# SixLabors/ZlibStream

Measured on AMD Instinct MI355X. Metric: deflate MB/s (input) at level 6, 64 MiB buffers, higher is better.
Workload: dtype u8; 1 GPU; english64: 1 x 67108864-byte pseudo-random-English (Zipf words of alice29.txt) buffer per GPU, level 6, zlib framing, inputs resident in HBM; level=6, buffer_bytes=67108864, buffers_per_gpu=1, compressed_bytes=27425826, parallelism=independent buffers, 1 GPU(s), no collective in the data path

## Files before the change

### zlibstream_amd/csrc/zs_core.h

```cpp
#pragma once
#include <stdint.h>
#include <vector>

#if defined(__HIPCC__)
#include <hip/hip_runtime.h>
#define ZS_HD __host__ __device__ __forceinline__
#define ZS_HD_NOINLINE __host__ __device__
#else
#define ZS_HD inline
#define ZS_HD_NOINLINE
#endif

namespace zs {

constexpr int kMinMatch = 3;
constexpr int kMaxMatch = 258;
constexpr int kMinLookahead = kMaxMatch + kMinMatch + 1;
constexpr int kWSize = 32768;
constexpr int kWMask = kWSize - 1;
constexpr int kWindowSize = 2 * kWSize;
constexpr int kMaxDist = kWSize - kMinLookahead;
constexpr int kSlideAt = kWindowSize - kMinLookahead;
constexpr int kHashBits = 15;
constexpr int kHashSize = 1 << kHashBits;
// ... 836 lines not shown
        if (nextlen == 0) max_count = 138, min_count = 3;
        else if (curlen == nextlen) max_count = 6, min_count = 3;
        else max_count = 7, min_count = 4;
    }
}

template <class Put>
ZS_HD_NOINLINE inline void emit_dyn_header(const TreeWork &w, Put &put) {
    int lcodes = w.l_max_code + 1, dcodes = w.d_max_code + 1, blcodes = w.max_blindex + 1;
    put((unsigned)(lcodes - 257), 5);
    put((unsigned)(dcodes - 1), 5);
    put((unsigned)(blcodes - 4), 4);
    for (int rank = 0; rank < blcodes; rank++) put(w.bltree[bl_order(rank)].dl, 3);
    emit_tree_rle(w.ltree, lcodes - 1, w.bltree, put);
    emit_tree_rle(w.dtree, dcodes - 1, w.bltree, put);
}

ZS_HD unsigned zlib_header(int level) {
    unsigned header = (8u + (7u << 4)) << 8;
    unsigned lf = (((unsigned)(level - 1)) & 0xFF) >> 1;
    if (lf > 3) lf = 3;
    header |= lf << 6;
    header += 31 - (header % 31);
    return header;
}

constexpr uint32_t kAdlerBase = 65521;
ZS_HD uint32_t adler_combine(uint32_t a1, uint32_t a2, uint64_t len2) {
    uint32_t rem = (uint32_t)(len2 % kAdlerBase);
    uint32_t s1a = a1 & 0xFFFF, s2a = a1 >> 16, s1b = a2 & 0xFFFF, s2b = a2 >> 16;
// ... 173 lines not shown
```

### zlibstream_amd/csrc/zs_device.h

```cpp
#pragma once
#include <cstddef>
#include "zs_core.h"
#include "zs_lit_engine.h"
#include "zs_fast_sweep.h"
#include "zs_rle.h"

namespace zs {

constexpr int kMatchTile = 16384;
constexpr int kMatchBack = 32512;
constexpr int kMatchFwd = 272;
constexpr int kMatchLdsBytes = kMatchBack + kMatchTile + kMatchFwd;
constexpr int kMatchLdsLinks = kMatchBack + kMatchTile;
constexpr int kMatchLds = kMatchLdsBytes + 2 * kMatchLdsLinks;
constexpr int kAdlerPiece = 65536;

constexpr int64_t kScratchWindow = 0;
constexpr int64_t kScratchHead = 66560;
constexpr int64_t kScratchPrev = kScratchHead + 2 * kHashSize;
constexpr int64_t kScratchHead32 = kScratchPrev + 2 * kWSize;
constexpr int64_t kScratchBytes = kScratchHead32 + 4 * kHashSize;

struct StreamDesc {
    const uint8_t *in;
// ... 81 lines not shown
    uint32_t adler;
    int32_t status;
    int64_t end_bits;
    int32_t r_seg, r_slot, r_kfired, r_kslot;
    uint32_t r_total;
    int32_t r_ncut;
    int32_t r_cut_e[8], r_cut_done[8];
    int32_t deferred, r_scan;
    int32_t r_cutidx;
    int32_t nc[2], cuts_same, cut_diff_idx, cut_diff_pos;
    int32_t poison;
    int32_t spec_run_tiles, spec_ok, spec_wrong;
    int32_t body_bad;
    int64_t body_bits;
};
constexpr uint32_t kSpecBail = 1u << 30;
ZS_HD uint32_t spec_pack(int guess, int exit_slot, int count, bool bail) {
    return (uint32_t)guess | ((uint32_t)exit_slot << 9) | ((uint32_t)count << 18) | (bail ? kSpecBail : 0u);
}
ZS_HD int spec_guess(uint32_t r) { return (int)(r & 0x1FF); }
ZS_HD int spec_exit(uint32_t r) { return (int)((r >> 9) & 0x1FF); }
ZS_HD int spec_count(uint32_t r) { return (int)((r >> 18) & 0xFFF); }
constexpr int kSpecMinInput = 1 << 20;
constexpr int kSpecLenBits = 10;
constexpr int kSpecWarm = 128;
constexpr int kSpecRunsDen = 8;
struct K5Spec {
    uint32_t *rec;
    uint32_t *base;
    int len_bits, warm, corrupt;
// ... 32 lines not shown
```

### zlibstream_amd/csrc/zs_engine.hip

```cpp
#include <hip/hip_runtime.h>

#include <algorithm>
#include <cstdio>
#include <cstdlib>
#include <cstring>
#include <functional>
#include <string>
#include <thread>
#include <vector>

#define ZS_BUILDING_LIBRARY
#include "../../include/zsgpu.h"
#include "zs_kernels.hip"
#include "zs_inflate_par.hip"
#include "zs_inflate_tok.hip"
#include "zs_png.hip"
#include "zs_crc32.hip"
#include "zs_gzip.hip"
#include "zs_zip.hip"
#include "zs_tiff.hip"
#include "zs_exr.hip"
#include "zs_chunk.hip"
#include "zs_plan.h"

// ... 39 lines not shown
    int fast_fallbacks = 0;
    int round_runs = 0;
    int cut_rounds = 0;
    int lit_fallbacks = 0;
    int spec_streams = 0, spec_fallbacks = 0, spec_wrong_chunks = 0;
    int spec_periodic = 0;
    int64_t dbg_blk_off = 0, dbg_chunk_off = 0, dbg_nchunks = 0, dbg_spec_n = 0, dbg_n_spec = 0;
    int64_t lit_engine_bytes = 0;
    std::vector<int64_t> inf_used;
    int64_t *inf_probe = nullptr;
    int inf_lane_streams = 0;
    int inf_wave_streams = 0;
    int64_t png_segments = 0;
    int fast_rounds = 0;
    bool no_rounds_once = false;
    int last_op = 0;
    hipEvent_t ev[kStCount + 1] = {};
    double stage_ms[kStCount] = {};
    uint32_t *crc_tab = nullptr;
    DevBuf sd, st, work, link, mm, maps, chunk_far, segmap, supmap, seg_entry, seg_symbase, seg_stale, entry, symbase, stale, syms, blk_end, blk_top, blocks, trees, info, tile_bits, pieces, scratch,
        stage_in, stage_out, wr, inf_desc, inf_state, par_ps, par_st, par_work, par_cbits, par_ccnt, par_surv, par_scnt, par_cands, par_tabs, par_toktabs, par_toks, par_ctoks, par_tokstat, par_tails, par_retry, par_fxtab, par_blocks, par_cells,
        par_windows, par_fail, run_syms, run_bits, run_scratch, run_outs, run_fail, adl_tr, adl_res, plan_blk, ins_bits, mm_bak, cut_pos, cut_bkt, win_groups, win_sg, win_maps, win_entries, persist_bak, resume_flag, rle_tiles, own_in, fr_chunks, fr_meta, fr_planes, fr_prov, fr_base, fr_counters, spec_rec, spec_flags, spec_syms;
    uint32_t *crc32_tab = nullptr;
    DevBuf png[kBufPngCount];
    hipEvent_t ev_png[2] = {};
    bool resume_poisoned = false;
    void *pinned = nullptr;
    size_t pinned_cap = 0;
    void *pin_io = nullptr;
    size_t pin_io_cap = 0;
// ... 81 lines not shown
T *dev(DevBuf &b) {
    return (T *)b.p;
}


struct RunOpts : PlanRun {
    int64_t end_bits = 0;
};

struct LaunchEnv {
    bool no_plan_reuse = getenv("ZS_NO_PLAN_REUSE") != nullptr, no_supmap = getenv("ZS_NO_SUPMAP") != nullptr;
    bool no_defer = getenv("ZS_NO_DEFER") != nullptr, force_rounds = getenv("ZS_FORCE_ROUNDS") != nullptr;
    bool tail_serial = getenv("ZS_TAIL_SERIAL") != nullptr, tail_fork = getenv("ZS_TAIL_FORK") != nullptr, fast_no_probe = getenv("ZS_FAST_NO_PROBE") != nullptr;
    bool no_whole_runs = getenv("ZS_NO_WHOLE_RUNS") != nullptr, whole_runs = getenv("ZS_WHOLE_RUNS") != nullptr;
    bool no_split_backend = getenv("ZS_NO_SPLIT_BACKEND") != nullptr;
    bool debug = getenv("ZS_DEBUG") != nullptr, debug_cuts = getenv("ZS_DEBUG_CUTS") != nullptr, debug_fa = getenv("ZS_DEBUG_FA") != nullptr;
    const char *debug_chain = getenv("ZS_DEBUG_CHAIN"), *debug_chain_want = getenv("ZS_DEBUG_CHAIN_WANT");
    int k5_ahead = getenv("ZS_K5_AHEAD") ? atoi(getenv("ZS_K5_AHEAD")) : 1;
    int spec_corrupt = getenv("ZS_SPEC_CORRUPT") ? atoi(getenv("ZS_SPEC_CORRUPT")) : -1;
    static bool host_times() {
        static const bool v = getenv("ZS_HOST_TIMES") != nullptr;
        return v;
    }
    static const char *eb_tiles() {
        static const char *const v = getenv("ZS_EB_TILES");
        return v;
    }
};
struct RoundsEnv {
    int max_rounds = getenv("ZS_FR_MAX_ROUNDS") ? atoi(getenv("ZS_FR_MAX_ROUNDS")) : 0;
// ... 35 lines not shown
    LaunchEnv env;
    FoldedWrites folded;
    PlanArgs pa;
    bool any_writes = false, no_rounds_this_call = false, plan_hit = false, plan_keep = false;
    double ht_plan = 0, ht_launched = 0;
    const StreamDesc *d_sd = nullptr;
    StreamState *d_st = nullptr, *hst = nullptr;
    const uint2 *d_work = nullptr;
    bool prof = false;
    K5Spec k5s{};
    int spec_ok_streams = 0;
    bool need_maps = true, spec_ran = false;
    bool fork_recorded = false;
    bool tail_late = false, tail_serial = false, use_sup = false;
    bool split = false;
    int defer_mode = 0, cut_stride = 0;
    bool done = false, answer = false;

    double ht_us() const { return std::chrono::duration<double, std::micro>(std::chrono::steady_clock::now() - ht0).count(); }
    const uint2 *work(int list) const { return d_work + lay.work[list]; }
    void mark(int i) {
        if (prof) (void)hipEventRecord(c->ev[i], stream);
    }
    bool rerun(int force_seq_, bool rounds_, const std::vector<uint8_t> *force_lit_) {
        c->lit_engine_bytes -= pl.lit_bytes;
        done = true;
        return answer = run_pipeline(c, n, in, in_len, out, out_cap, out_len, status, level, strategy, hash_variant, stream, writes, force_seq_, ro, rounds_, force_lit_);
    }
    void launch_tail(hipStream_t on) {
        hipLaunchKernelGGL(zs_tail_kernel, dim3((unsigned)n), dim3(1024), kTailLds, on, d_sd, d_st, dev<uint16_t>(c->link),
// ... 37 lines not shown

bool DeflateCall::begin() {
    for (int i = 0; i < n; i++) {
        out_len[i] = 0;
        if (status) status[i] = ZS_STREAM_ERROR;
    }
    for (int i = 0; i < n && writes; i++) any_writes = any_writes || writes[i] != nullptr;
    if (any_writes && n > 1)
        for (int i = 0; i < n; i++)
            if (ro || (writes[i] && writes[i]->flushing())) {
                c->err = "flush modes and incremental runs take one stream a call";
                return false;
            }
    no_rounds_this_call = c->no_rounds_once;
    c->no_rounds_once = false;
    c->fast_rounds = 0;
    c->plan_reused = 0;
    bool flush_any = false;
    for (int i = 0; i < n && any_writes; i++)
        if (const WriteSpec *wr = writes[i]) flush_any = flush_any || wr->flushing() || wr->flush.size() != wr->ends.size();
    plan_keep = !ro && !rounds && !force_lit && !no_rounds_this_call && force_seq == 0 && level != 0 && !flush_any && !env.no_plan_reuse;
    if (plan_keep) {
        plan_key_fill(pc.probe, n, in_len, out_cap, level, strategy, hash_variant, force_seq, ro != nullptr, rounds, force_lit != nullptr, no_rounds_this_call,
                      any_writes ? writes : nullptr, penv);
        plan_hit = pc.valid && pc.gen == c->plan_gen && !pc.in_flight && plan_key_equal(pc.key, pc.probe);
    }
    if (!plan_hit) pc.valid = false, pc.dual_saved = false, c->plan_gen++;
    writes = fold_rle_writes(folded, n, in_len, writes, any_writes, level, strategy, ro != nullptr, penv);
    pa.n = n, pa.in = in, pa.in_len = in_len, pa.out = out, pa.out_cap = out_cap, pa.level = level, pa.strategy = strategy;
    pa.writes = writes, pa.force_seq = force_seq, pa.ro = ro, pa.rounds = rounds, pa.force_lit = force_lit, pa.no_rounds = no_rounds_this_call;
// ... 365 lines not shown
    };
    tiles([&](dim3 tg, int s0) { hipLaunchKernelGGL(zs_rle_starts_kernel, tg, dim3(256), 0, stream, d_sd, rt, s0); });
    hipLaunchKernelGGL(zs_rle_scan_kernel, dim3((unsigned)n), dim3(1024), 0, stream, d_sd, rt);
    tiles([&](dim3 tg, int s0) {
        hipLaunchKernelGGL(zs_rle_pass_kernel<0>, tg, dim3(256), 0, stream, d_sd, rt, dev<uint32_t>(c->syms), dev<int32_t>(c->blk_end), dev<int32_t>(c->blk_top), s0);
    });
    hipLaunchKernelGGL(zs_rle_sums_kernel, dim3((unsigned)n), dim3(1024), 0, stream, d_sd, d_st, rt);
    tiles([&](dim3 tg, int s0) {
        hipLaunchKernelGGL(zs_rle_pass_kernel<1>, tg, dim3(256), 0, stream, d_sd, rt, dev<uint32_t>(c->syms), dev<int32_t>(c->blk_end), dev<int32_t>(c->blk_top), s0);
    });
    return true;
}

bool DeflateCall::tails_and_symbols() {
    const bool beside_k5 = need_maps && (!pl.w_segs.empty() || !pl.w_chunks.empty());
    if (!tail_late && !tail_serial && (n < 64 || penv.no_live_list) && !env.no_split_backend && pl.n_runs == 0 && !beside_k5) {
        int64_t longest = 0;
        for (int i = 0; i < n; i++) longest = std::max(longest, in_len[i]);
        split = longest >= kBlockSyms;
    }
    if (!tail_late && !tail_serial) {
        if (!fork_recorded || need_maps) ZS_HIP(c, hipEventRecord(c->ev_fork, stream));
        ZS_HIP(c, hipStreamWaitEvent(c->aux, c->ev_fork, 0));
        launch_tail(c->aux);
        if (split && prof) (void)hipEventRecord(c->ev_part1[0], c->aux);
        if (!split) ZS_HIP(c, hipEventRecord(c->ev_join, c->aux));
    }
    if (!pl.w_segs.empty() && need_maps)
        hipLaunchKernelGGL(zs_expand_kernel, dim3((unsigned)((pl.w_segs.size() + 63) / 64)), dim3(64), 0, stream, d_sd, d_st,
                           work(kWSegs), (int)pl.w_segs.size(), dev<uint2>(c->mm), dev<uint16_t>(c->link),
                           dev<uint32_t>(c->maps), dev<uint16_t>(c->seg_entry), dev<uint32_t>(c->seg_symbase),
// ... 78 lines not shown
                       dev<uint32_t>(c->run_syms), dev<FastRunOut>(c->run_outs), dev<uint32_t>(c->syms), dev<int32_t>(c->blk_end),
                       dev<int32_t>(c->blk_top));
    hipLaunchKernelGGL(zs_fast_blocks_kernel, dim3((unsigned)n), dim3(64), 0, stream, d_sd, d_st, dev<FastRunOut>(c->run_outs),
                       dev<int32_t>(c->blk_end), dev<int32_t>(c->blk_top), dev<BlockRec>(c->blocks), n);
    return true;
}

bool DeflateCall::blocks_and_bits() {
    const int trees_threads = pl.w_blocks.size() > 8192 ? 128 : 256;
    if (n >= 64 && !penv.no_live_list) {
        int32_t *const d_live = (int32_t *)((uint8_t *)c->sd.p + lay.sd_bytes);
        hipLaunchKernelGGL(zs_live_scan_kernel, dim3(1), dim3(1024), 0, stream, d_st, n, d_live);
        hipLaunchKernelGGL(zs_live_fill_kernel, dim3((unsigned)((pl.w_blocks.size() + 255) / 256)), dim3(256), 0, stream, d_live, n,
                           (uint32_t)pl.w_blocks.size(), dev<uint2>(c->work) + lay.work[kWBlocks]);
    }
    auto trees = [&](hipStream_t on, int part) {
        hipLaunchKernelGGL(zs_trees_kernel, dim3((unsigned)pl.w_blocks.size()), dim3(trees_threads), 0, on, d_sd, d_st, work(kWBlocks), dev<uint32_t>(c->syms),
                           dev<BlockRec>(c->blocks), dev<TreeWork>(c->trees), dev<BlockInfo>(c->info), dev<int32_t>(c->tile_bits), strategy, level, part);
    };
    auto offsets = [&](hipStream_t on, int part) {
        hipLaunchKernelGGL(zs_offsets_kernel, dim3((unsigned)n), dim3(256), 0, on, d_sd, d_st, dev<BlockRec>(c->blocks), dev<BlockInfo>(c->info),
                           dev<TreeWork>(c->trees), dev<uint32_t>(c->pieces), level, n, part);
    };
    trees(stream, split ? kPartBody : kPartAll);
    mark(11);
    ZS_HIP(c, hipStreamWaitEvent(stream, c->ev_pre, 0));
    offsets(stream, split ? kPartBody : kPartAll);
    mark(12);
    if (split) ZS_HIP(c, hipEventRecord(c->ev_part0, stream));
    int eb_tiles = kEbTiles;
    if (level != 0) {
        int64_t longest = 0;
        for (int i = 0; i < n; i++) longest = std::max(longest, in_len[i]);
        eb_tiles = (int)std::min<int64_t>(kEbTiles, (longest + 1) / kEbTile + 1);
    }
    if (env.eb_tiles()) eb_tiles = std::max(1, std::min(kEbTiles, atoi(env.eb_tiles())));
    auto emit_bits = [&](hipStream_t on, int part) {
        hipLaunchKernelGGL(zs_emit_bits_kernel, dim3((unsigned)pl.w_blocks.size(), (unsigned)(1 + eb_tiles)), dim3(256), 0, on, d_sd, d_st, work(kWBlocks),
                           dev<uint32_t>(c->syms), dev<BlockRec>(c->blocks), dev<TreeWork>(c->trees), dev<BlockInfo>(c->info), dev<int32_t>(c->tile_bits), part);
    };
    emit_bits(stream, split ? kPartBody : kPartAll);
    mark(13);
    if (split) {
        trees(c->aux, kPartRest);
        ZS_HIP(c, hipStreamWaitEvent(c->aux, c->ev_part0, 0));
        offsets(c->aux, kPartRest);
        emit_bits(c->aux, kPartRest);
        if (prof) (void)hipEventRecord(c->ev_part1[1], c->aux);
        ZS_HIP(c, hipEventRecord(c->ev_join, c->aux));
        ZS_HIP(c, hipStreamWaitEvent(stream, c->ev_join, 0));
    }
    ZS_HIP(c, hipGetLastError());
    hst = (StreamState *)c->pinned;
    ZS_HIP(c, hipMemcpyAsync(hst, d_st, sizeof(StreamState) * (size_t)n, hipMemcpyDeviceToHost, stream));
// ... 77 lines not shown
                c->resume_poisoned = true;
                return false;
            }
            c->lit_fallbacks++;
            return rerun(force_seq, false, &fl);
        }
    }
    if (!ro && !rounds) {
        bool gave_up = false;
        for (int i = 0; i < n; i++) gave_up = gave_up || hst[i].deferred == 1;
        if (gave_up) {
            ZS_HIP(c, hipStreamSynchronize(c->aux));
            c->round_runs++;
            if (!run_cut_rounds()) return false;
            return rerun(force_seq, true, force_lit);
        }
    }
    if (ro) ro->end_bits = hst[0].end_bits;
    bool all_ok = true;
    for (int i = 0; i < n; i++) {
        out_len[i] = hst[i].out_len;
        if (status) status[i] = hst[i].status;
        if (hst[i].status != 0 && all_ok) {
            c->err = hst[i].status == ZS_BUF_ERROR ? "buffer error"
                                                   : "stored block larger than the reference's pending buffer (the managed engine throws here)";
            all_ok = false;
        }
    }
    return all_ok;
}
// ... 221 lines not shown
const char *zs_ctx_last_error(const zs_ctx *c) { return c ? c->err.c_str() : "no context"; }

int64_t zs_deflate_bound(int64_t n) { return n + (n >> 3) + 1024; }

void zs_ctx_set_profiling(zs_ctx *c, int enable) {
    if (c) c->profiling = enable != 0;
}
int zs_ctx_stage_count(const zs_ctx *) { return kStCount; }
int64_t zs_ctx_counter(const zs_ctx *c, const char *name) {
    if (!c || !name) return -1;
    const std::string k(name);
    if (k == "fast_rounds") return c->fast_rounds;
    if (k == "fast_fallbacks") return c->fast_fallbacks;
    if (k == "round_runs") return c->round_runs;
    if (k == "cut_rounds") return c->cut_rounds;
    if (k == "lit_fallbacks") return c->lit_fallbacks;
    if (k == "lit_engine_bytes") return c->lit_engine_bytes;
    if (k == "spec_streams") return c->spec_streams;
    if (k == "spec_fallbacks") return c->spec_fallbacks;
    if (k == "spec_periodic") return c->spec_periodic;
    if (k == "spec_wrong_chunks") return c->spec_wrong_chunks;
    if (k == "plan_reused") return c->plan_reused;
    if (k == "inf_lane_streams") return c->inf_lane_streams;
    if (k == "inf_wave_streams") return c->inf_wave_streams;
    if (k == "png_segments") return c->png_segments;
    return -1;
}

int64_t zs_ctx_debug_read(zs_ctx *c, const char *name, void *out, int64_t cap) {
    if (!c || !name || !out || !c->st.p) return -1;
// ... 787 lines not shown
```

### zlibstream_amd/csrc/zs_kernels.hip

```cpp
#include <hip/hip_runtime.h>

#include <type_traits>

#include "zs_device.h"
#include "zs_png.h"

namespace zs {

typedef uint32_t __attribute__((aligned(1))) u32u;
typedef uint64_t __attribute__((aligned(1))) u64u;
typedef const __attribute__((address_space(1))) uint8_t *gcbytes;
typedef __attribute__((address_space(1))) uint8_t *gbytes_w;
__device__ __forceinline__ gcbytes as_global(const uint8_t *p) { return (gcbytes)(uintptr_t)p; }
__device__ __forceinline__ gbytes_w as_global(uint8_t *p) { return (gbytes_w)(uintptr_t)p; }
typedef const __attribute__((address_space(1))) uint32_t __attribute__((aligned(1))) *gcu32u;
typedef const __attribute__((address_space(1))) uint64_t __attribute__((aligned(1))) *gcu64u;
__device__ __forceinline__ uint32_t g_u32_bytes(gcbytes p) {
    return (uint32_t)p[0] | ((uint32_t)p[1] << 8) | ((uint32_t)p[2] << 16) | ((uint32_t)p[3] << 24);
}
typedef uint32_t u32x4 __attribute__((ext_vector_type(4)));
typedef const __attribute__((address_space(1))) u32x4 *gcu32x4;
__device__ __forceinline__ uint32_t lds_u32(const uint8_t *base, int idx) {
    const uint32_t *q = (const uint32_t *)(base + (idx & ~3));
    return __builtin_amdgcn_alignbyte(q[1], q[0], (uint32_t)idx & 3u);
// ... 1979 lines not shown
    }
    if (cut < 0) return;
#pragma unroll
    for (int d = 32; d >= 1; d >>= 1) before += __shfl_xor(before, d, 64);
    if (lane != 0) return;
    const ChunkCtx cx = spec_chunk_ctx(s, c, sp.len_bits);
    const int64_t start = spec_first_start(cx.cs, spec_guess(r)) + before;
    const bool odd = cx.m != 0 && slab[sp.stride - 1] == (uint32_t)cut;
    const uint32_t bi = (base + (uint32_t)cut) / kBlockSyms;
    blk_end[s.blk_off + bi] = (int32_t)spec_sym_end(start, slab[cut]);
    blk_top[s.blk_off + bi] = (int32_t)spec_sym_top(start, odd);
}

enum { kPartAll = -1, kPartBody = 0, kPartRest = 1 };
__device__ __forceinline__ int stream_body_blocks(int part, const StreamDesc &s, const StreamState &ss) {
    if (part == kPartAll) return 0;
    const bool splits = s.wr_flush == nullptr && s.n_wr <= 1 && s.final_run && !s.resume && !s.cont && !s.cont_bits && s.fast_runs == 0 &&
                        s.plan_nblk == 0 && !ss.deferred;
    return splits ? (int)(ss.body_syms / kBlockSyms) : 0;
}

__global__ __launch_bounds__(256) void zs_body_blocks_kernel(const StreamDesc *sd, const StreamState *st, const int32_t *blk_end,
                                                             const int32_t *blk_top, BlockRec *blocks, uint32_t *syms, int part) {
    const StreamDesc s = sd[blockIdx.x];
    if (s.fast_runs > 0 || st[blockIdx.x].deferred) return;
    const int nb0 = stream_body_blocks(part, s, st[blockIdx.x]);
    if (part == kPartBody && nb0 == 0) return;
    if (s.resume)
        for (uint32_t i = threadIdx.x; i < s.start_syms; i += blockDim.x) syms[s.sym_off + i] = s.persist->syms[i];
    const int nb_body = (int)(st[blockIdx.x].body_syms / kBlockSyms);
    BlockRec *blk = blocks + s.blk_off;
    for (int i = threadIdx.x; i < (part == kPartRest && nb0 > 0 ? 0 : nb_body); i += blockDim.x) {
        int64_t start = i ? blk_end[s.blk_off + i - 1] : (s.resume ? s.start_block : 0);
        int64_t end = blk_end[s.blk_off + i];
// ... 735 lines not shown
    while (lo < hi) {
        const int mid = (lo + hi + 1) >> 1;
        if (live_pre[mid] <= (int32_t)g) lo = mid;
        else hi = mid - 1;
    }
    work[g] = make_uint2((uint32_t)lo, g - (uint32_t)live_pre[lo]);
}

#ifdef ZS_BS_PROF
#define BS_PF(i) { const long long now_ = wall_clock64(); pf[i] += now_ - pf_t; pf_t = now_; }
#else
#define BS_PF(i)
#endif
typedef u32x4 __attribute__((aligned(4))) u32x4a4;
typedef u32x4 __attribute__((aligned(8))) u32x4a8;
__global__ __launch_bounds__(256) void zs_trees_kernel(const StreamDesc *sd, const StreamState *st, const uint2 *work,
                                                       const uint32_t *syms, const BlockRec *blocks, TreeWork *trees,
                                                       BlockInfo *info, int32_t *tile_bits, int strategy, int level, int part) {
    __shared__ __attribute__((aligned(16))) TreeWork tw;
    __shared__ SideTree sw;
    __shared__ uint32_t hl[kLCodes], hd[kDCodes];
    __shared__ uint32_t hk[kHeapSize + 8];
    __shared__ uint32_t pd[kHeapSize + 1], nc[16];
    __shared__ uint32_t hk2[SideTree::kHeap + 8], pd2[SideTree::kHeap + 1], nc2[16];
    __shared__ uint32_t sh_tile[2 * kEbTiles];
    __shared__ int sh_type;
#ifdef ZS_BS_PROF
    long long pf[8] = {0, 0, 0, 0, 0, 0, 0, 0}, pf_t = wall_clock64();
#endif
    uint2 w = work[blockIdx.x];
    if (w.x == kNoWork || st[w.x].deferred) return;
    const StreamDesc s = sd[w.x];
    const int b = (int)w.y;
    const int nb0 = stream_body_blocks(part, s, st[w.x]);
    if (part == kPartBody ? b >= nb0 : (b < nb0 || b >= st[w.x].nblocks)) return;
    const BlockRec r = blocks[s.blk_off + b];
    if (level == 0 && r.nsyms == 0 && s.plan_nblk > 0) {
        if (threadIdx.x == 0) {
            BlockInfo bi;
            bi.type = r.can_store ? 0 : 1;
            bi.bits = r.can_store ? 0 : 10;
            bi.bit_start = 0;
            info[s.blk_off + b] = bi;
        }
        return;
// ... 126 lines not shown
        constexpr int nw = (int)(sizeof(TreeWork) / 4);
        for (int i = tid; i < nw / 4; i += nthr) dv[i] = src4[i];
        uint32_t *dst = (uint32_t *)&trees[s.blk_off + b];
        const uint32_t *src = (const uint32_t *)&tw;
        if (tid < (nw & 3)) dst[(nw & ~3) + tid] = src[(nw & ~3) + tid];
    }
    BS_PF(6);
    const int type = sh_type;
    if (tiled && type != 0 && tid < kEbTiles) tile_bits[(int64_t)(s.blk_off + b) * kEbTiles + tid] = (int32_t)sh_tile[(type == 2 ? 0 : kEbTiles) + tid];
#ifdef ZS_BS_PROF
    BS_PF(7);
    if (lane == 0 && wave < 2 && (blockIdx.x & 255) == 7)
        printf("BSPROF K7 block %d wave %d nsyms %d type %d ticks(100MHz): zero=%lld histogram=%lld fill=%lld ltree+scan/wait=%lld dtree+scan=%lld bltree+type (tile bits beside it)=%lld copy-out=%lld tile bits out=%lld\n",
               (int)blockIdx.x, wave, r.nsyms, type, pf[0], pf[1], pf[2], pf[3], pf[4], pf[5], pf[6], pf[7]);
#endif
}
#undef BS_PF

__device__ __forceinline__ void or_bits(uint8_t *out, int64_t pos, uint64_t v, int nbits) {
    if (nbits == 0) return;
    uint32_t *w = (uint32_t *)((uintptr_t)(out + (pos >> 3)) & ~(uintptr_t)3);
    int sh = (int)(pos - ((int64_t)((uint8_t *)w - out) << 3));
    uint64_t lo = v << sh;
    uint32_t w0 = (uint32_t)lo, w1 = (uint32_t)(lo >> 32);
    uint32_t w2 = sh ? (uint32_t)(v >> (64 - sh)) : 0;
    if (w0) atomicOr(w, w0);
    if (w1) atomicOr(w + 1, w1);
    if (w2) atomicOr(w + 2, w2);
}
struct OrBitsAt {
// ... 194 lines not shown
struct LdsBitPut {
    uint32_t *w;
    uint32_t pos;
    __device__ void put64(uint64_t v, int nbits) {
        if (nbits == 0) return;
        const uint32_t k = pos >> 5, sh = pos & 31;
        const uint64_t lo = v << sh;
        const uint32_t w0 = (uint32_t)lo, w1 = (uint32_t)(lo >> 32), w2 = sh ? (uint32_t)(v >> (64 - sh)) : 0;
        if (w0) atomicOr(&w[k], w0);
        if (w1) atomicOr(&w[k + 1], w1);
        if (w2) atomicOr(&w[k + 2], w2);
        pos += (uint32_t)nbits;
    }
    __device__ void operator()(unsigned value, int nbits) { put64(value, nbits); }
};
#ifdef ZS_BS_PROF
#define BS_PF(i) { const long long now_ = wall_clock64(); pf[i] += now_ - pf_t; pf_t = now_; }
#else
#define BS_PF(i)
#endif
__global__ __launch_bounds__(256) void zs_emit_bits_kernel(const StreamDesc *sd, const StreamState *st, const uint2 *work,
                                                           const uint32_t *syms, const BlockRec *blocks, const TreeWork *trees,
                                                           const BlockInfo *info, const int32_t *tile_bits, int split_part) {
    __shared__ uint32_t lt[kLCodes], dt[kDCodes];
    __shared__ uint32_t obuf[kEbWords];
    __shared__ uint32_t wsum[4];
    __shared__ uint32_t sh_bits;
#ifdef ZS_BS_PROF
    long long pf[4] = {0, 0, 0, 0}, pf_t = wall_clock64();
#endif
    uint2 w = work[blockIdx.x];
    if (w.x == kNoWork || st[w.x].deferred) return;
    const StreamDesc s = sd[w.x];
    const int b = (int)w.y;
    const int nb0 = stream_body_blocks(split_part, s, st[w.x]);
    if (split_part == kPartBody ? b >= nb0 : (b >= st[w.x].nblocks || st[w.x].status != 0)) return;
    const BlockRec r = blocks[s.blk_off + b];
    const BlockInfo bi = info[s.blk_off + b];
    if (b < nb0) {
        const int64_t end_byte = bi.type == 0 ? ((bi.bit_start + 3 + 7) >> 3) + 4 + r.stored_len : (bi.bit_start + bi.bits + 7) >> 3;
        const bool fits = end_byte + 12 <= s.out_cap;
        if (fits != (split_part == kPartBody)) return;
    }
    uint8_t *out = s.out;
    const int tid = threadIdx.x, lane = lane_id(), wave = tid >> 6;
    const int part = (int)blockIdx.y, ntl = (int)gridDim.y - 1;
// ... 26 lines not shown
            if (k == 0 || k == nw - 1) {
                if (v) atomicOr(g + k, v);
            } else {
                g[k] = v;
            }
            obuf[k] = 0;
        }
        __syncthreads();
    };
    const TreeWork &tw = trees[s.blk_off + b];
    if (part == 0) {
        if (bi.type == 1) {
            if (tid == 0) or_bits(out, bi.bit_start, 2u + (unsigned)(r.eof & 1), 3);
            return;
        }
        constexpr int kHdrWords = 160, kTwWords = (int)(sizeof(TreeWork) / 4);
        static_assert(kHdrWords + kTwWords <= kEbWords && sizeof(TreeWork) % 4 == 0, "the header and a TreeWork fit obuf");
        for (int i = tid; i < kHdrWords; i += 256) obuf[i] = 0;
        for (int i = tid; i < kTwWords; i += 256) obuf[kHdrWords + i] = ((const uint32_t *)&tw)[i];
        __syncthreads();
        if (tid == 0) {
            LdsBitPut put{obuf, (uint32_t)(cur0 & 31)};
            put(4u + (unsigned)(r.eof & 1), 3);
            emit_dyn_header(*(const TreeWork *)(obuf + kHdrWords), put);
            sh_bits = put.pos - (uint32_t)(cur0 & 31);
        }
        __syncthreads();
        BS_PF(1);
        flush(cur0, sh_bits);
#ifdef ZS_BS_PROF
        BS_PF(3);
        if (tid == 0 && (blockIdx.x & 255) == 7) printf("BSPROF K9 block %d header ticks(100MHz): header=%lld flush=%lld\n", (int)blockIdx.x, pf[1], pf[3]);
#endif
        return;
    }
    const int total = r.nsyms + 1;
    const int ntiles = (total + kEbTile - 1) / kEbTile;
    if (part - 1 >= ntiles) return;
    if (bi.type == 2) {
        for (int i = tid; i < kLCodes; i += 256) lt[i] = (uint32_t)tw.ltree[i].fc | ((uint32_t)tw.ltree[i].dl << 16);
// ... 54 lines not shown
                    acc >>= fl;
                    fill -= fl;
                }
            }
        }
        if (fill) put.put64(acc, fill);
        __syncthreads();
        BS_PF(2);
        flush(cur, mine);
        BS_PF(3);
    }
#ifdef ZS_BS_PROF
    if (tid == 0 && (blockIdx.x & 255) == 7)
        printf("BSPROF K9 block %d part %d ticks(100MHz): tables=%lld tile=%lld flush=%lld\n", (int)blockIdx.x, part, pf[0], pf[2], pf[3]);
#endif
}

__global__ __launch_bounds__(256) void zs_adler_kernel(const StreamDesc *sd, const uint2 *work, uint32_t *pieces) {
    __shared__ uint64_t ra[256], rb[256];
    uint2 w = work[blockIdx.x];
    const StreamDesc s = sd[w.x];
    int64_t beg = (int64_t)w.y * kAdlerPiece;
    int64_t len = (int64_t)s.n - beg;
    if (len > kAdlerPiece) len = kAdlerPiece;
    const gcbytes p = as_global(s.in) + beg;
    int64_t o = (int64_t)threadIdx.x * 256;
    int64_t lt = len - o;
    if (lt > 256) lt = 256;
    if (lt < 0) lt = 0;
    uint64_t a = 0, bsum = 0;
// ... 229 lines not shown
```

Measured before the change: 16450 MB/s.

## Launch rest-part trees/emit kernels per stream and emit dynamic headers wave-parallel

```diff
diff --git a/zlibstream_amd/csrc/zs_core.h b/zlibstream_amd/csrc/zs_core.h
--- a/zlibstream_amd/csrc/zs_core.h
+++ b/zlibstream_amd/csrc/zs_core.h
@@ -874,6 +874,47 @@
     for (int rank = 0; rank < blcodes; rank++) put(w.bltree[bl_order(rank)].dl, 3);
     emit_tree_rle(w.ltree, lcodes - 1, w.bltree, put);
     emit_tree_rle(w.dtree, dcodes - 1, w.bltree, put);
+}
+
+template <class F>
+ZS_HD void header_run_tokens(int v, int R, F &&f) {
+    if (v == 0) {
+        for (; R >= 138; R -= 138) f(18, 127u, 7);
+        if (R >= 11) f(18, (unsigned)(R - 11), 7);
+        else if (R >= 3) f(17, (unsigned)(R - 3), 3);
+        else
+            for (; R > 0; R--) f(0, 0u, 0);
+        return;
+    }
+    if (R >= 4) {
+        const int g = R < 7 ? R : 7;
+        f(v, 0u, 0);
+        f(16, (unsigned)(g - 4), 2);
+        for (R -= g; R >= 6; R -= 6) f(16, 3u, 2);
+        if (R >= 3) f(16, (unsigned)(R - 3), 2), R = 0;
+    }
+    for (; R > 0; R--) f(v, 0u, 0);
+}
+template <class BL>
+ZS_HD int header_run_bits(int v, int R, const BL &bl) {
+    int bits = 0;
+    header_run_tokens(v, R, [&](int code, unsigned, int xb) { bits += (int)(bl(code) >> 16) + xb; });
+    return bits;
+}
+template <class BL, class Put>
+ZS_HD void emit_header_run(int v, int R, const BL &bl, Put &put) {
+    header_run_tokens(v, R, [&](int code, unsigned extra, int xb) {
+        const uint32_t e = bl(code);
+        put((e & 0xFFFFu) | (extra << (e >> 16)), (int)(e >> 16) + xb);
+    });
+}
+template <class Put>
+inline void emit_tree_runs(const CtData *tree, int max_code, const CtData *bltree, Put &put) {
+    auto bl = [&](int c) { return (uint32_t)bltree[c].fc | ((uint32_t)bltree[c].dl << 16); };
+    for (int s = 0, e; s <= max_code; s = e) {
+        for (e = s + 1; e <= max_code && tree[e].dl == tree[s].dl; e++) {}
+        emit_header_run(tree[s].dl, e - s, bl, put);
+    }
 }
 
 ZS_HD unsigned zlib_header(int level) {
diff --git a/zlibstream_amd/csrc/zs_device.h b/zlibstream_amd/csrc/zs_device.h
--- a/zlibstream_amd/csrc/zs_device.h
+++ b/zlibstream_amd/csrc/zs_device.h
@@ -119,6 +119,12 @@
     int32_t body_bad;
     int64_t body_bits;
 };
+
+ZS_HD int stream_rest_bound(const StreamDesc &s, const StreamState &ss) {
+    const bool splits = s.wr_flush == nullptr && s.n_wr <= 1 && s.final_run && !s.resume && !s.cont && !s.cont_bits && s.fast_runs == 0 &&
+                        s.plan_nblk == 0 && !ss.deferred;
+    return splits ? (int)(ss.body_syms / 16383u) : 0;
+}
 constexpr uint32_t kSpecBail = 1u << 30;
 ZS_HD uint32_t spec_pack(int guess, int exit_slot, int count, bool bail) {
     return (uint32_t)guess | ((uint32_t)exit_slot << 9) | ((uint32_t)count << 18) | (bail ? kSpecBail : 0u);
diff --git a/zlibstream_amd/csrc/zs_engine.hip b/zlibstream_amd/csrc/zs_engine.hip
--- a/zlibstream_amd/csrc/zs_engine.hip
+++ b/zlibstream_amd/csrc/zs_engine.hip
@@ -77,6 +77,8 @@
     int64_t png_segments = 0;
     int fast_rounds = 0;
     bool no_rounds_once = false;
+    bool no_split_once = false;
+    int rest_reruns = 0;
     int last_op = 0;
     hipEvent_t ev[kStCount + 1] = {};
     double stage_ms[kStCount] = {};
@@ -188,6 +190,7 @@
     bool tail_serial = getenv("ZS_TAIL_SERIAL") != nullptr, tail_fork = getenv("ZS_TAIL_FORK") != nullptr, fast_no_probe = getenv("ZS_FAST_NO_PROBE") != nullptr;
     bool no_whole_runs = getenv("ZS_NO_WHOLE_RUNS") != nullptr, whole_runs = getenv("ZS_WHOLE_RUNS") != nullptr;
     bool no_split_backend = getenv("ZS_NO_SPLIT_BACKEND") != nullptr;
+    int rest_slots = getenv("ZS_REST_SLOTS") ? atoi(getenv("ZS_REST_SLOTS")) : 0;
     bool debug = getenv("ZS_DEBUG") != nullptr, debug_cuts = getenv("ZS_DEBUG_CUTS") != nullptr, debug_fa = getenv("ZS_DEBUG_FA") != nullptr;
     const char *debug_chain = getenv("ZS_DEBUG_CHAIN"), *debug_chain_want = getenv("ZS_DEBUG_CHAIN_WANT");
     int k5_ahead = getenv("ZS_K5_AHEAD") ? atoi(getenv("ZS_K5_AHEAD")) : 1;
@@ -253,6 +256,9 @@
     bool fork_recorded = false;
     bool tail_late = false, tail_serial = false, use_sup = false;
     bool split = false;
+    bool no_split_this_call = false;
+    int rest_slots = 0;
+    bool rest_by_streams = false;
     int defer_mode = 0, cut_stride = 0;
     bool done = false, answer = false;
 
@@ -320,6 +326,8 @@
             }
     no_rounds_this_call = c->no_rounds_once;
     c->no_rounds_once = false;
+    no_split_this_call = c->no_split_once;
+    c->no_split_once = false;
     c->fast_rounds = 0;
     c->plan_reused = 0;
     bool flush_any = false;
@@ -715,7 +723,7 @@
 
 bool DeflateCall::tails_and_symbols() {
     const bool beside_k5 = need_maps && (!pl.w_segs.empty() || !pl.w_chunks.empty());
-    if (!tail_late && !tail_serial && (n < 64 || penv.no_live_list) && !env.no_split_backend && pl.n_runs == 0 && !beside_k5) {
+    if (!tail_late && !tail_serial && (n < 64 || penv.no_live_list) && !env.no_split_backend && !no_split_this_call && pl.n_runs == 0 && !beside_k5) {
         int64_t longest = 0;
         for (int i = 0; i < n; i++) longest = std::max(longest, in_len[i]);
         split = longest >= kBlockSyms;
@@ -824,9 +832,26 @@
         hipLaunchKernelGGL(zs_live_fill_kernel, dim3((unsigned)((pl.w_blocks.size() + 255) / 256)), dim3(256), 0, stream, d_live, n,
                            (uint32_t)pl.w_blocks.size(), dev<uint2>(c->work) + lay.work[kWBlocks]);
     }
+    rest_slots = kRestSlots;
+    if (split) {
+        const StreamState none{};
+        for (int i = 0; i < n; i++) {
+            const StreamDesc &s = pl.sd[(size_t)i];
+            StreamState some = none;
+            some.body_syms = kBlockSyms;
+            const bool may_split = stream_rest_bound(s, some) > 0 && (s.body_end >= 0 || s.fv_end >= 0 || s.rle_end >= 0);
+            if (!may_split) rest_slots = std::max(rest_slots, (int)std::min<int64_t>(s.max_blocks, 65534));
+        }
+    }
+    if (env.rest_slots > 0 && !ro) rest_slots = std::min(env.rest_slots, 65534);
+    rest_by_streams = split && (int64_t)n * rest_slots <= (int64_t)pl.w_blocks.size();
     auto trees = [&](hipStream_t on, int part) {
-        hipLaunchKernelGGL(zs_trees_kernel, dim3((unsigned)pl.w_blocks.size()), dim3(trees_threads), 0, on, d_sd, d_st, work(kWBlocks), dev<uint32_t>(c->syms),
-                           dev<BlockRec>(c->blocks), dev<TreeWork>(c->trees), dev<BlockInfo>(c->info), dev<int32_t>(c->tile_bits), strategy, level, part);
+        if (part == kPartRest && rest_by_streams)
+            hipLaunchKernelGGL(zs_trees_rest_kernel, dim3((unsigned)n, (unsigned)rest_slots), dim3(trees_threads), 0, on, d_sd, d_st, dev<uint32_t>(c->syms),
+                               dev<BlockRec>(c->blocks), dev<TreeWork>(c->trees), dev<BlockInfo>(c->info), dev<int32_t>(c->tile_bits), strategy, level, part);
+        else
+            hipLaunchKernelGGL(zs_trees_kernel, dim3((unsigned)pl.w_blocks.size()), dim3(trees_threads), 0, on, d_sd, d_st, work(kWBlocks), dev<uint32_t>(c->syms),
+                               dev<BlockRec>(c->blocks), dev<TreeWork>(c->trees), dev<BlockInfo>(c->info), dev<int32_t>(c->tile_bits), strategy, level, part);
     };
     auto offsets = [&](hipStream_t on, int part) {
         hipLaunchKernelGGL(zs_offsets_kernel, dim3((unsigned)n), dim3(256), 0, on, d_sd, d_st, dev<BlockRec>(c->blocks), dev<BlockInfo>(c->info),
@@ -846,8 +871,12 @@
     }
     if (env.eb_tiles()) eb_tiles = std::max(1, std::min(kEbTiles, atoi(env.eb_tiles())));
     auto emit_bits = [&](hipStream_t on, int part) {
-        hipLaunchKernelGGL(zs_emit_bits_kernel, dim3((unsigned)pl.w_blocks.size(), (unsigned)(1 + eb_tiles)), dim3(256), 0, on, d_sd, d_st, work(kWBlocks),
-                           dev<uint32_t>(c->syms), dev<BlockRec>(c->blocks), dev<TreeWork>(c->trees), dev<BlockInfo>(c->info), dev<int32_t>(c->tile_bits), part);
+        if (part == kPartRest && rest_by_streams)
+            hipLaunchKernelGGL(zs_emit_bits_rest_kernel, dim3((unsigned)n, (unsigned)(1 + eb_tiles), (unsigned)(rest_slots + 1)), dim3(256), 0, on, d_sd, d_st,
+                               dev<uint32_t>(c->syms), dev<BlockRec>(c->blocks), dev<TreeWork>(c->trees), dev<BlockInfo>(c->info), dev<int32_t>(c->tile_bits), part);
+        else
+            hipLaunchKernelGGL(zs_emit_bits_kernel, dim3((unsigned)pl.w_blocks.size(), (unsigned)(1 + eb_tiles)), dim3(256), 0, on, d_sd, d_st, work(kWBlocks),
+                               dev<uint32_t>(c->syms), dev<BlockRec>(c->blocks), dev<TreeWork>(c->trees), dev<BlockInfo>(c->info), dev<int32_t>(c->tile_bits), part);
     };
     emit_bits(stream, split ? kPartBody : kPartAll);
     mark(13);
@@ -955,6 +984,20 @@
             c->round_runs++;
             if (!run_cut_rounds()) return false;
             return rerun(force_seq, true, force_lit);
+        }
+    }
+    if (rest_by_streams) {
+        for (int i = 0; i < n; i++) {
+            if ((int64_t)hst[i].nblocks - stream_rest_bound(pl.sd[(size_t)i], hst[i]) <= rest_slots) continue;
+            ZS_HIP(c, hipStreamSynchronize(c->aux));
+            if (ro && ro->resume) {
+                c->err = "the resumed run has more blocks behind its body than the back end's second part was launched for";
+                c->resume_poisoned = true;
+                return false;
+            }
+            c->no_split_once = true;
+            c->rest_reruns++;
+            return rerun(force_seq, rounds, force_lit);
         }
     }
     if (ro) ro->end_bits = hst[0].end_bits;
@@ -1206,6 +1249,7 @@
     if (k == "fast_fallbacks") return c->fast_fallbacks;
     if (k == "round_runs") return c->round_runs;
     if (k == "cut_rounds") return c->cut_rounds;
+    if (k == "rest_reruns") return c->rest_reruns;
     if (k == "lit_fallbacks") return c->lit_fallbacks;
     if (k == "lit_engine_bytes") return c->lit_engine_bytes;
     if (k == "spec_streams") return c->spec_streams;
diff --git a/zlibstream_amd/csrc/zs_kernels.hip b/zlibstream_amd/csrc/zs_kernels.hip
--- a/zlibstream_amd/csrc/zs_kernels.hip
+++ b/zlibstream_amd/csrc/zs_kernels.hip
@@ -2017,10 +2017,7 @@
 
 enum { kPartAll = -1, kPartBody = 0, kPartRest = 1 };
 __device__ __forceinline__ int stream_body_blocks(int part, const StreamDesc &s, const StreamState &ss) {
-    if (part == kPartAll) return 0;
-    const bool splits = s.wr_flush == nullptr && s.n_wr <= 1 && s.final_run && !s.resume && !s.cont && !s.cont_bits && s.fast_runs == 0 &&
-                        s.plan_nblk == 0 && !ss.deferred;
-    return splits ? (int)(ss.body_syms / kBlockSyms) : 0;
+    return part == kPartAll ? 0 : stream_rest_bound(s, ss);
 }
 
 __global__ __launch_bounds__(256) void zs_body_blocks_kernel(const StreamDesc *sd, const StreamState *st, const int32_t *blk_end,
@@ -2786,9 +2783,8 @@
 #endif
 typedef u32x4 __attribute__((aligned(4))) u32x4a4;
 typedef u32x4 __attribute__((aligned(8))) u32x4a8;
-__global__ __launch_bounds__(256) void zs_trees_kernel(const StreamDesc *sd, const StreamState *st, const uint2 *work,
-                                                       const uint32_t *syms, const BlockRec *blocks, TreeWork *trees,
-                                                       BlockInfo *info, int32_t *tile_bits, int strategy, int level, int part) {
+__device__ __forceinline__ void trees_block(const StreamDesc *sd, const StreamState *st, const uint2 w, const uint32_t *syms, const BlockRec *blocks,
+                                            TreeWork *trees, BlockInfo *info, int32_t *tile_bits, int strategy, int level, int part) {
     __shared__ __attribute__((aligned(16))) TreeWork tw;
     __shared__ SideTree sw;
     __shared__ uint32_t hl[kLCodes], hd[kDCodes];
@@ -2800,7 +2796,6 @@
 #ifdef ZS_BS_PROF
     long long pf[8] = {0, 0, 0, 0, 0, 0, 0, 0}, pf_t = wall_clock64();
 #endif
-    uint2 w = work[blockIdx.x];
     if (w.x == kNoWork || st[w.x].deferred) return;
     const StreamDesc s = sd[w.x];
     const int b = (int)w.y;
@@ -2957,6 +2952,21 @@
         printf("BSPROF K7 block %d wave %d nsyms %d type %d ticks(100MHz): zero=%lld histogram=%lld fill=%lld ltree+scan/wait=%lld dtree+scan=%lld bltree+type (tile bits beside it)=%lld copy-out=%lld tile bits out=%lld\n",
                (int)blockIdx.x, wave, r.nsyms, type, pf[0], pf[1], pf[2], pf[3], pf[4], pf[5], pf[6], pf[7]);
 #endif
+}
+constexpr int kRestSlots = 2;
+__device__ __forceinline__ uint2 rest_block(const StreamDesc *sd, const StreamState *st, int part, int slot) {
+    const int si = (int)blockIdx.x;
+    const int b = stream_body_blocks(part, sd[si], st[si]) + slot;
+    return b < 0 || b >= st[si].nblocks ? make_uint2(kNoWork, 0u) : make_uint2((uint32_t)si, (uint32_t)b);
+}
+__global__ __launch_bounds__(256) void zs_trees_kernel(const StreamDesc *sd, const StreamState *st, const uint2 *work,
+                                                       const uint32_t *syms, const BlockRec *blocks, TreeWork *trees,
+                                                       BlockInfo *info, int32_t *tile_bits, int strategy, int level, int part) {
+    trees_block(sd, st, work[blockIdx.x], syms, blocks, trees, info, tile_bits, strategy, level, part);
+}
+__global__ __launch_bounds__(256) void zs_trees_rest_kernel(const StreamDesc *sd, const StreamState *st, const uint32_t *syms, const BlockRec *blocks,
+                                                            TreeWork *trees, BlockInfo *info, int32_t *tile_bits, int strategy, int level, int part) {
+    trees_block(sd, st, rest_block(sd, st, part, (int)blockIdx.y), syms, blocks, trees, info, tile_bits, strategy, level, part);
 }
 #undef BS_PF
 
@@ -3181,14 +3191,47 @@
     }
     __device__ void operator()(unsigned value, int nbits) { put64(value, nbits); }
 };
+__device__ uint32_t header_tree_wave(const uint32_t *len, int n, const uint32_t *bl, uint32_t *runs, uint32_t *obuf, uint32_t pos,
+                                     int lane) {
+    int nruns = 0;
+    for (int base = 0; base < n; base += 64) {
+        const int i = base + lane;
+        const bool start = i < n && (i == 0 || len[i] != len[i - 1]);
+        const uint64_t m = __ballot(start);
+        if (start) runs[nruns + __builtin_popcountll(m & lanemask_lt())] = (uint32_t)i;
+        nruns += __builtin_popcountll(m);
+    }
+    __threadfence_block();
+    auto blf = [&](int c) { return bl[c]; };
+    for (int base = 0; base < nruns; base += 64) {
+        const int k = base + lane;
+        int v = 0, R = 0;
+        if (k < nruns) {
+            const int s = (int)runs[k];
+            R = (k + 1 < nruns ? (int)runs[k + 1] : n) - s;
+            v = (int)len[s];
+        }
+        const uint32_t mine = (uint32_t)header_run_bits(v, R, blf);
+        uint32_t inc = mine;
+#pragma unroll
+        for (int off = 1; off < 64; off <<= 1) {
+            const uint32_t o = (uint32_t)__shfl_up((int)inc, off);
+            if (lane >= off) inc += o;
+        }
+        LdsBitPut put{obuf, pos + inc - mine};
+        emit_header_run(v, R, blf, put);
+        pos += (uint32_t)__shfl((int)inc, 63);
+    }
+    __threadfence_block();
+    return pos;
+}
 #ifdef ZS_BS_PROF
 #define BS_PF(i) { const long long now_ = wall_clock64(); pf[i] += now_ - pf_t; pf_t = now_; }
 #else
 #define BS_PF(i)
 #endif
-__global__ __launch_bounds__(256) void zs_emit_bits_kernel(const StreamDesc *sd, const StreamState *st, const uint2 *work,
-                                                           const uint32_t *syms, const BlockRec *blocks, const TreeWork *trees,
-                                                           const BlockInfo *info, const int32_t *tile_bits, int split_part) {
+__device__ __forceinline__ void emit_bits_block(const StreamDesc *sd, const StreamState *st, const uint2 w, const uint32_t *syms, const BlockRec *blocks,
+                                                const TreeWork *trees, const BlockInfo *info, const int32_t *tile_bits, int split_part) {
     __shared__ uint32_t lt[kLCodes], dt[kDCodes];
     __shared__ uint32_t obuf[kEbWords];
     __shared__ uint32_t wsum[4];
@@ -3196,7 +3239,6 @@
 #ifdef ZS_BS_PROF
     long long pf[4] = {0, 0, 0, 0}, pf_t = wall_clock64();
 #endif
-    uint2 w = work[blockIdx.x];
     if (w.x == kNoWork || st[w.x].deferred) return;
     const StreamDesc s = sd[w.x];
     const int b = (int)w.y;
@@ -3253,16 +3295,26 @@
             if (tid == 0) or_bits(out, bi.bit_start, 2u + (unsigned)(r.eof & 1), 3);
             return;
         }
-        constexpr int kHdrWords = 160, kTwWords = (int)(sizeof(TreeWork) / 4);
-        static_assert(kHdrWords + kTwWords <= kEbWords && sizeof(TreeWork) % 4 == 0, "the header and a TreeWork fit obuf");
+        constexpr int kHdrWords = 160;
+        static_assert(kHdrWords + 32 + kLCodes <= kEbWords && kBlCodes <= 32, "the header, the bit-length tree and the run starts fit obuf");
+        uint32_t *const blw = obuf + kHdrWords, *const runs = blw + 32;
+        const int lcodes = tw.l_max_code + 1, dcodes = tw.d_max_code + 1, blcodes = tw.max_blindex + 1;
         for (int i = tid; i < kHdrWords; i += 256) obuf[i] = 0;
-        for (int i = tid; i < kTwWords; i += 256) obuf[kHdrWords + i] = ((const uint32_t *)&tw)[i];
-        __syncthreads();
-        if (tid == 0) {
-            LdsBitPut put{obuf, (uint32_t)(cur0 & 31)};
-            put(4u + (unsigned)(r.eof & 1), 3);
-            emit_dyn_header(*(const TreeWork *)(obuf + kHdrWords), put);
-            sh_bits = put.pos - (uint32_t)(cur0 & 31);
+        for (int i = tid; i < lcodes && i < kLCodes; i += 256) lt[i] = tw.ltree[i].dl;
+        if (tid < dcodes && tid < kDCodes) dt[tid] = tw.dtree[tid].dl;
+        if (tid < kBlCodes) blw[tid] = (uint32_t)tw.bltree[tid].fc | ((uint32_t)tw.bltree[tid].dl << 16);
+        __syncthreads();
+        if (wave == 0) {
+            const uint32_t p0 = (uint32_t)(cur0 & 31);
+            LdsBitPut put{obuf, p0};
+            if (lane == 0)
+                put(4u + (unsigned)(r.eof & 1) + ((unsigned)(lcodes - 257) << 3) + ((unsigned)(dcodes - 1) << 8) + ((unsigned)(blcodes - 4) << 13), 17);
+            put.pos = p0 + 17 + 3 * (uint32_t)lane;
+            if (lane < blcodes && lane < kBlCodes) put(blw[bl_order(lane)] >> 16, 3);
+            uint32_t pos = p0 + 17 + 3 * (uint32_t)blcodes;
+            pos = header_tree_wave(lt, lcodes < kLCodes ? lcodes : kLCodes, blw, runs, obuf, pos, lane);
+            pos = header_tree_wave(dt, dcodes < kDCodes ? dcodes : kDCodes, blw, runs, obuf, pos, lane);
+            if (lane == 0) sh_bits = pos - p0;
         }
         __syncthreads();
         BS_PF(1);
@@ -3347,6 +3399,15 @@
     if (tid == 0 && (blockIdx.x & 255) == 7)
         printf("BSPROF K9 block %d part %d ticks(100MHz): tables=%lld tile=%lld flush=%lld\n", (int)blockIdx.x, part, pf[0], pf[2], pf[3]);
 #endif
+}
+__global__ __launch_bounds__(256) void zs_emit_bits_kernel(const StreamDesc *sd, const StreamState *st, const uint2 *work,
+                                                           const uint32_t *syms, const BlockRec *blocks, const TreeWork *trees,
+                                                           const BlockInfo *info, const int32_t *tile_bits, int split_part) {
+    emit_bits_block(sd, st, work[blockIdx.x], syms, blocks, trees, info, tile_bits, split_part);
+}
+__global__ __launch_bounds__(256) void zs_emit_bits_rest_kernel(const StreamDesc *sd, const StreamState *st, const uint32_t *syms, const BlockRec *blocks,
+                                                                const TreeWork *trees, const BlockInfo *info, const int32_t *tile_bits, int split_part) {
+    emit_bits_block(sd, st, rest_block(sd, st, split_part, (int)blockIdx.z - 1), syms, blocks, trees, info, tile_bits, split_part);
 }
 
 __global__ __launch_bounds__(256) void zs_adler_kernel(const StreamDesc *sd, const uint2 *work, uint32_t *pieces) {
```

New measurement: 16630 MB/s, median of 6. 1.1% higher.
